# arielgabizon/barretenberg

Hardware: AMD Instinct MI355X
Metric: BN254 G1 MSM points/sec at n=2^20 (Fr NTT elems/sec in 'ntt') (higher is better)
Workload: dtype u32x9 (256-bit Montgomery, 29-bit limbs)

## Files before the change

barretenberg_amd/csrc/msm.hip:

```cpp
#include <hip/hip_runtime.h>

#include <algorithm>
#include <mutex>
#include <stdint.h>
#include <stdio.h>
#include <stdlib.h>
#include <string.h>
#include <vector>

#include "bbgpu_internal.h"
#include "g1.hpp"
#include "g1_quad.hpp"
#include "host_g1.hpp"

namespace bbgpu {

using Fr = FrP;
#define FRONT_PRIO() __builtin_amdgcn_s_setprio(2)
constexpr int TAIL_PRIO = 3;
constexpr int SCALAR_BITS = 254;
constexpr int MSM_MAX_C = 16;
constexpr int MSM_THREADS = 256;

__device__ __forceinline__ void ld8(const uint32_t* p, uint32_t (&w)[8])
{
    const uint4* q = reinterpret_cast<const uint4*>(p);
    uint4 a = q[0], b = q[1];
    w[0] = a.x; w[1] = a.y; w[2] = a.z; w[3] = a.w;
    w[4] = b.x; w[5] = b.y; w[6] = b.z; w[7] = b.w;
}
__device__ __forceinline__ void ld16(const uint32_t* p, uint32_t (&w)[16])
{
    const uint4* q = reinterpret_cast<const uint4*>(p);
#pragma unroll
    for (int i = 0; i < 4; i++) {
        uint4 a = q[i];
        w[4 * i] = a.x; w[4 * i + 1] = a.y; w[4 * i + 2] = a.z; w[4 * i + 3] = a.w;
    }
}
__device__ __forceinline__ void st32(uint32_t* p, const uint32_t (&w)[32])
{
    uint4* q = reinterpret_cast<uint4*>(p);
#pragma unroll
    for (int i = 0; i < 8; i++) q[i] = make_uint4(w[4 * i], w[4 * i + 1], w[4 * i + 2], w[4 * i + 3]);
}
__device__ __forceinline__ void ld32(const uint32_t* p, uint32_t (&w)[32])
{
    const uint4* q = reinterpret_cast<const uint4*>(p);
#pragma unroll
    for (int i = 0; i < 8; i++) {
        uint4 a = q[i];
        w[4 * i] = a.x; w[4 * i + 1] = a.y; w[4 * i + 2] = a.z; w[4 * i + 3] = a.w;
    }
}

struct WinLayout {
    uint16_t off[66];
};
static WinLayout make_layout(int c, bool balanced)
{
    WinLayout LO{};
    const int W = msm_num_windows(c);
    if (!balanced) {
        for (int w = 0; w <= W; w++) LO.off[w] = (uint16_t)(c * w);
        return LO;
    }
    const int base = SCALAR_BITS / W, rem = SCALAR_BITS - base * W;
    int bit = 0;
    for (int w = 0; w < W; w++) {
        LO.off[w] = (uint16_t)bit;
        bit += base + (w < rem ? 1 : 0);
    }
    LO.off[W] = (uint16_t)bit;
    return LO;
}
__global__ void srs_convert_kernel(const uint32_t* __restrict__ table, uint32_t* __restrict__ srs, uint32_t n, uint32_t stride_words)
{
    const uint32_t i = blockIdx.x * blockDim.x + threadIdx.x;
    if (i >= n) return;
    uint32_t w[16];
    ld16(table + (size_t)i * stride_words, w);
    AffineV<2> a;
    load_affine_m256(a, w);
    uint32_t o[16];
    store_affine_m261(o, a.x, a.y);
    uint4* q = reinterpret_cast<uint4*>(srs + (size_t)i * 16);
#pragma unroll
    for (int k = 0; k < 4; k++) q[k] = make_uint4(o[4 * k], o[4 * k + 1], o[4 * k + 2], o[4 * k + 3]);
}

// ... 71 lines not shown
    set_infinity(acc);
    for (uint32_t d = 0; d < 256; d++) {
        uint32_t o[32];
        store_xyzz(o, acc);
        st32(tab + ((size_t)w * 256 + d) * 32, o);
        Xyzz t;
        add(t, acc, base);
        acc = t;
    }
}
__device__ __forceinline__ Fe<Fq, 1, 2> fq_inverse(const Fe<Fq, 1, 2>& a)
{
    const uint64_t e[4] = { Fq::P64[0] - 2, Fq::P64[1], Fq::P64[2], Fq::P64[3] };
    return pow_u256<Fq>(a, e);
}
__global__ void srs_gen_points_kernel(const uint32_t* __restrict__ tab, Limbs9 x261, uint32_t* __restrict__ srs, uint32_t n, uint32_t first)
{
    const uint32_t i = blockIdx.x * blockDim.x + threadIdx.x;
    if (i >= n) return;
    Fe<Fr, 1, 2> s = fe_one<Fr>(), b = fe_from<Fr>(x261.d);
    for (uint32_t e = first + i; e; e >>= 1) {
        if (e & 1) s = mul(s, b);
        b = sqr(b);
    }
    uint32_t k[8];
    {
        FeT<Fr> one_raw = fe_zero<Fr>();
        one_raw.d[0] = 1;
        to_canonical(mul(s, one_raw), k);
    }
    Xyzz acc;
    set_infinity(acc);
    for (uint32_t w = 0; w < 32; w++) {
        const uint32_t d = (k[w >> 2] >> ((w & 3) * 8)) & 0xff;
        if (d) {
            uint32_t pw[32];
            ld32(tab + ((size_t)w * 256 + d) * 32, pw);
            Xyzz q;
            load_xyzz(q, pw);
            Xyzz t;
            add(t, acc, q);
            acc = t;
        }
    }
    auto inv = fq_inverse(mul(acc.zz, acc.zzz));
    auto izz = mul(inv, acc.zzz), izzz = mul(inv, acc.zz);
    uint32_t o[16];
    store_affine_m261(o, mul(acc.x, izz), mul(acc.y, izzz));
    uint4* q = reinterpret_cast<uint4*>(srs + (size_t)i * 16);
#pragma unroll
    for (int t = 0; t < 4; t++) q[t] = make_uint4(o[4 * t], o[4 * t + 1], o[4 * t + 2], o[4 * t + 3]);
}

struct ScalarSets {
    const uint32_t* p[MSM_MAX_JOBS];
};
template <class DT> struct DigitTraits { static constexpr bool wide = false; };
template <> struct DigitTraits<uint16_t> { static constexpr bool wide = true; };
template <class DT> __device__ __forceinline__ int load_digit(const DT* __restrict__ dg, const unsigned long long* __restrict__ sg, uint32_t i)
{
    if constexpr (DigitTraits<DT>::wide) {
        const int u = dg[i];
        return ((sg[i >> 6] >> (i & 63u)) & 1ull) ? -u - 1 : u;
    } else {
        return dg[i];
    }
}
template <class DT> __device__ __forceinline__ void load_digits8(const DT* __restrict__ dg, const unsigned long long* __restrict__ sg, uint32_t i8, int (&d)[8])
{
    const uint4 q = *reinterpret_cast<const uint4*>(dg + i8);
    const uint32_t w[4] = { q.x, q.y, q.z, q.w };
    if constexpr (DigitTraits<DT>::wide) {
        const uint32_t sb = reinterpret_cast<const uint8_t*>(sg)[i8 >> 3];
#pragma unroll
        for (int k = 0; k < 8; k++) {
            const int u = (int)((w[k >> 1] >> (16 * (k & 1))) & 0xffffu);
            d[k] = ((sb >> k) & 1u) ? -u - 1 : u;
        }
    } else {
#pragma unroll
        for (int k = 0; k < 8; k++) d[k] = (int)(int16_t)(w[k >> 1] >> (16 * (k & 1)));
    }
}
template <class DT> __global__ void __launch_bounds__(MSM_THREADS) msm_digits_kernel(ScalarSets sets, DT* __restrict__ digits_all, unsigned long long* __restrict__ signs_all,
                                                               uint32_t n, WinLayout LO, uint32_t num_windows, uint32_t wb, uint32_t we)
{
    FRONT_PRIO();
    const uint32_t i = blockIdx.x * blockDim.x + threadIdx.x;
    if (i >= n) return;
    const uint32_t* __restrict__ scalars = sets.p[blockIdx.y];
    DT* __restrict__ digits = digits_all + (size_t)blockIdx.y * num_windows * n;
    const uint32_t s64 = (n + 63) >> 6;
    unsigned long long* __restrict__ signs = signs_all + (size_t)blockIdx.y * num_windows * s64;
    uint32_t w[8], k[9];
    ld8(scalars + (size_t)i * 8, w);
    to_canonical(exact_limbs(mul(unpack<Fr>(w), fe_from<Fr>(Fr::M256_TO_PLAIN))), w);
#pragma unroll
    for (int j = 0; j < 8; j++) k[j] = w[j];
    k[8] = 0;
    uint32_t carry = 0;
    for (uint32_t win = 0; win < we; win++) {
        const uint32_t bit = LO.off[win], sz = LO.off[win + 1] - bit, j = bit >> 5, s = bit & 31;
        const uint32_t half = 1u << (sz - 1), mask = (1u << sz) - 1;
        uint32_t v = 0;
        if (j < 8) {
            v = k[j] >> s;
            if (s + sz > 32) v |= k[j + 1] << (32 - s);
        }
        v = (v & mask) + carry;
        carry = (win + 1 < num_windows && v >= half) ? 1u : 0u;
        const int32_t d = (int32_t)v - (int32_t)(carry << sz);
        if (win >= wb) {
            if constexpr (DigitTraits<DT>::wide) {
                const unsigned long long neg = __ballot(d < 0);
                digits[(size_t)win * n + i] = (DT)(d < 0 ? -d - 1 : d);
                if ((threadIdx.x & 63u) == 0) signs[(size_t)win * s64 + (i >> 6)] = neg;
            } else {
                digits[(size_t)win * n + i] = (DT)d;
            }
        }
    }
}

constexpr int SORT_THREADS = 1024;
constexpr uint32_t SORT_MAX_LB = 7;
constexpr uint32_t SORTB_MAX_PARTS = 8;
constexpr uint32_t SORTB_SPLIT_MIN = 1u << 16;

__device__ __forceinline__ bool wave_keys_heavy(bool valid, uint32_t key)
{
    const uint64_t vm = __ballot(valid);
    if (!vm) return false;
    const uint32_t k0 = __builtin_amdgcn_readlane(key, __ffsll((unsigned long long)vm) - 1);
    return 4 * __popcll(__ballot(valid && key == k0)) >= __popcll(vm);
}
__device__ __forceinline__ uint32_t lds_inc_dedup(uint32_t* ctr, uint32_t key, bool heavy)
{
    if (!heavy) return atomicAdd(&ctr[key], 1u);
    const uint32_t lane = __lane_id();
    uint64_t todo = __ballot(1);
    uint32_t res = 0;
    for (int it = 0; it < 4 && todo; it++) {
        const int leader = __ffsll((unsigned long long)todo) - 1;
        const uint32_t kk = __builtin_amdgcn_readlane(key, leader);
        const uint64_t m = __ballot(key == kk) & todo;
        uint32_t base = 0;
        if ((int)lane == leader) base = atomicAdd(&ctr[kk], (uint32_t)__popcll(m));
        base = __builtin_amdgcn_readlane(base, leader);
        if ((m >> lane) & 1ull) res = base + (uint32_t)__popcll(m & ((1ull << lane) - 1ull));
        todo &= ~m;
    }
    if ((todo >> lane) & 1ull) res = atomicAdd(&ctr[key], 1u);
    return res;
}

template <class DT> __global__ void __launch_bounds__(SORT_THREADS) __attribute__((amdgpu_num_vgpr(32))) sortA_hist_kernel(const DT* __restrict__ digits, const unsigned long long* __restrict__ signs, uint32_t* __restrict__ histA, uint32_t n,
                                                                uint32_t bins, uint32_t lb, uint32_t slices, uint32_t slice_len, uint32_t win0,
                                                                uint32_t wpg, uint32_t first_i0, uint32_t last_i1, uint32_t blo, uint32_t bcnt)
{
    FRONT_PRIO();
    __shared__ uint32_t lh[SORT_THREADS];
    const uint32_t s = blockIdx.x, wl = blockIdx.y;
    lh[threadIdx.x] = 0;
    __syncthreads();
    const uint32_t lo = s * slice_len, hi = min(n, lo + slice_len);
    const uint32_t s64 = (n + 63) >> 6;
    if ((n & 7u) == 0) {
        const uint32_t lo8 = lo & ~7u, bpw = lo < hi ? (((hi + 7u) & ~7u) - lo8) >> 3 : 0u;
        for (uint32_t u = threadIdx.x; u < wpg * bpw; u += SORT_THREADS) {
            const uint32_t k = u / bpw, i8 = lo8 + (u - k * bpw) * 8;
            const uint32_t klo = (k == 0) ? max(lo, first_i0) : lo, khi = (k + 1 == wpg) ? min(hi, last_i1) : hi;
            int d[8];
            load_digits8<DT>(digits + (size_t)(win0 + wl * wpg + k) * n, signs + (size_t)(win0 + wl * wpg + k) * s64, i8, d);
            const bool heavy = wave_keys_heavy(d[0] != 0, (uint32_t)((d[0] < 0 ? -d[0] : d[0]) - 1) >> lb);
#pragma unroll
            for (int j = 0; j < 8; j++)
                if (d[j] && i8 + j >= klo && i8 + j < khi) {
                    const uint32_t b = (uint32_t)((d[j] < 0 ? -d[j] : d[j]) - 1);
                    if (b - blo < bcnt) (void)lds_inc_dedup(lh, b >> lb, heavy);
                }
        }
    } else {
        for (uint32_t k = 0; k < wpg; k++) {
            const DT* dg = digits + (size_t)(win0 + wl * wpg + k) * n;
            const unsigned long long* sg = signs + (size_t)(win0 + wl * wpg + k) * s64;
            const uint32_t klo = (k == 0) ? max(lo, first_i0) : lo, khi = (k + 1 == wpg) ? min(hi, last_i1) : hi;
            for (uint32_t i = klo + threadIdx.x; i < khi; i += SORT_THREADS) {
                const int d = load_digit<DT>(dg, sg, i);
                if (d) {
                    const uint32_t b = (uint32_t)((d < 0 ? -d : d) - 1);
                    if (b - blo < bcnt) atomicAdd(&lh[b >> lb], 1u);
                }
            }
        }
    }
    __syncthreads();
    if (threadIdx.x < bins) histA[((size_t)wl * slices + s) * bins + threadIdx.x] = lh[threadIdx.x];
}

__global__ void __launch_bounds__(SORT_THREADS) sortA_colscan_kernel(uint32_t* __restrict__ histA, uint32_t* __restrict__ bintot, uint32_t bins,
                                                                   uint32_t slices)
{
    FRONT_PRIO();
    const uint32_t wl = blockIdx.y, lane = threadIdx.x & 63;
    const uint32_t bin = blockIdx.x * (SORT_THREADS / 64) + (threadIdx.x >> 6);
    if (bin >= bins) return;
    uint32_t* H = histA + (size_t)wl * slices * bins + bin;
    const uint32_t spp = (slices + 63) / 64;
    const uint32_t s0 = min(slices, lane * spp), s1 = min(slices, s0 + spp);
    uint32_t sum = 0;
    for (uint32_t s = s0; s < s1; s++) sum += H[(size_t)s * bins];
    uint32_t incl = sum;
#pragma unroll
    for (int off = 1; off < 64; off <<= 1) {
        const uint32_t v = __shfl_up(incl, off);
        if ((int)lane >= off) incl += v;
    }
    uint32_t run = incl - sum;
    for (uint32_t s = s0; s < s1; s++) {
        const uint32_t cnt = H[(size_t)s * bins];
        H[(size_t)s * bins] = run;
        run += cnt;
    }
    if (lane == 63) bintot[(size_t)wl * bins + bin] = incl;
}
__global__ void __launch_bounds__(SORT_THREADS) sortA_scan_kernel(const uint32_t* __restrict__ bintot, uint32_t* __restrict__ binstart,
                                                                uint32_t* __restrict__ totals, uint32_t bins, uint32_t* __restrict__ solo_bases,
                                                                uint32_t* __restrict__ solo_gstart_end)
{
    FRONT_PRIO();
    __shared__ uint32_t part[SORT_THREADS];
    const uint32_t wl = blockIdx.x, t = threadIdx.x;
    const uint32_t mine = t < bins ? bintot[(size_t)wl * bins + t] : 0;
    part[t] = mine;
    __syncthreads();
    for (uint32_t off = 1; off < SORT_THREADS; off <<= 1) {
        uint32_t v = t >= off ? part[t - off] : 0;
        __syncthreads();
        part[t] += v;
        __syncthreads();
    }
    if (t < bins) binstart[(size_t)wl * bins + t] = part[t] - mine;
    if (t == SORT_THREADS - 1) {
        totals[wl] = part[SORT_THREADS - 1];
        if (solo_bases) {
            solo_bases[0] = 0;
            solo_bases[1] = part[SORT_THREADS - 1];
            solo_gstart_end[0] = part[SORT_THREADS - 1];
            solo_gstart_end[1] = 0xffffffffu;
        }
    }
}
__global__ void sort_bases_kernel(const uint32_t* __restrict__ totals, uint32_t* __restrict__ bases, uint32_t* __restrict__ gstart_end, uint32_t nw)
{
    FRONT_PRIO();
    if (threadIdx.x == 0 && blockIdx.x == 0) {
        uint32_t run = 0;
        for (uint32_t w = 0; w < nw; w++) {
            bases[w] = run;
            run += totals[w];
        }
        bases[nw] = run;
        gstart_end[0] = run;
        gstart_end[1] = 0xffffffffu;
    }
}


template <class DT> __global__ void __launch_bounds__(SORT_THREADS) __attribute__((amdgpu_num_vgpr(32))) sortA_scatter_kernel(const DT* __restrict__ digits, const unsigned long long* __restrict__ signs, const uint32_t* __restrict__ cursorsA,
                                                                   const uint32_t* __restrict__ binstart, const uint32_t* __restrict__ bases,
                                                                   uint32_t* __restrict__ tmp, uint32_t n, uint32_t bins, uint32_t lb,
                                                                   uint32_t slices, uint32_t slice_len, uint32_t win0, uint32_t wpg,
                                                                   uint32_t idx_stride, uint32_t windows_per_job, uint32_t first_i0, uint32_t last_i1, uint32_t blo, uint32_t bcnt)
{
    FRONT_PRIO();
    __shared__ uint32_t lc[SORT_THREADS];
    const uint32_t s = blockIdx.x, wl = blockIdx.y;
    if (threadIdx.x < bins)
        lc[threadIdx.x] = cursorsA[((size_t)wl * slices + s) * bins + threadIdx.x] + binstart[(size_t)wl * bins + threadIdx.x] + bases[wl];
    __syncthreads();
    const uint32_t lo = s * slice_len, hi = min(n, lo + slice_len);
    const uint32_t lomask = (1u << lb) - 1;
    const uint32_t s64 = (n + 63) >> 6;
    if ((n & 7u) == 0) {
        const uint32_t lo8 = lo & ~7u, bpw = lo < hi ? (((hi + 7u) & ~7u) - lo8) >> 3 : 0u;
        for (uint32_t u = threadIdx.x; u < wpg * bpw; u += SORT_THREADS) {
            const uint32_t k = u / bpw, i8 = lo8 + (u - k * bpw) * 8;
            const uint32_t wabs = win0 + wl * wpg + k;
            const uint32_t row = (wabs % windows_per_job) * idx_stride;
            const uint32_t klo = (k == 0) ? max(lo, first_i0) : lo, khi = (k + 1 == wpg) ? min(hi, last_i1) : hi;
            int d[8];
            load_digits8<DT>(digits + (size_t)wabs * n, signs + (size_t)wabs * s64, i8, d);
#pragma unroll
            for (int j = 0; j < 8; j++) {
                if (d[j] && i8 + j >= klo && i8 + j < khi) {
                    const uint32_t b = (uint32_t)((d[j] < 0 ? -d[j] : d[j]) - 1);
                    if (b - blo < bcnt) {
                        const uint32_t pos = atomicAdd(&lc[b >> lb], 1u);
                        tmp[pos] = (row + i8 + j) | ((b & lomask) << 24) | (d[j] < 0 ? 0x80000000u : 0u);
                    }
                }
            }
        }
        return;
    }
    for (uint32_t k = 0; k < wpg; k++) {
        const uint32_t wabs = win0 + wl * wpg + k;
        const DT* dg = digits + (size_t)wabs * n;
        const unsigned long long* sg = signs + (size_t)wabs * s64;
        const uint32_t row = (wabs % windows_per_job) * idx_stride;
        const uint32_t klo = (k == 0) ? max(lo, first_i0) : lo, khi = (k + 1 == wpg) ? min(hi, last_i1) : hi;
        for (uint32_t i = klo + threadIdx.x; i < khi; i += SORT_THREADS) {
            const int d = load_digit<DT>(dg, sg, i);
            if (d) {
                const uint32_t b = (uint32_t)((d < 0 ? -d : d) - 1);
                if (b - blo < bcnt) {
                    const uint32_t pos = atomicAdd(&lc[b >> lb], 1u);
                    tmp[pos] = (row + i) | ((b & lomask) << 24) | (d < 0 ? 0x80000000u : 0u);
                }
            }
        }
    }
}

template <class DT> __global__ void __launch_bounds__(SORT_THREADS) __attribute__((amdgpu_waves_per_eu(8, 8))) sortA_scatter_staged_kernel(const DT* __restrict__ digits, const unsigned long long* __restrict__ signs, const uint32_t* __restrict__ cursorsA,
                                                                          const uint32_t* __restrict__ binstart, const uint32_t* __restrict__ bases,
                                                                          uint32_t* __restrict__ tmp, uint32_t n, uint32_t bins, uint32_t lb,
                                                                          uint32_t slices, uint32_t slice_len, uint32_t win0, uint32_t wpg,
                                                                          uint32_t idx_stride, uint32_t windows_per_job, uint32_t first_i0, uint32_t last_i1, uint32_t blo, uint32_t bcnt)
{
    FRONT_PRIO();
    constexpr uint32_t TILE = SORT_THREADS * 8;
    __shared__ uint32_t lc[SORT_THREADS];
    __shared__ uint32_t th[SORT_THREADS];
    __shared__ uint32_t dlt[SORT_THREADS];
    __shared__ uint32_t wsum[SORT_THREADS / 64 + 1];
    __shared__ uint32_t buf[TILE];
    __shared__ uint16_t bbin[TILE];
    const uint32_t s = blockIdx.x, wl = blockIdx.y, t = threadIdx.x, lane = t & 63, wave = t >> 6;
    lc[t] = t < bins ? cursorsA[((size_t)wl * slices + s) * bins + t] + binstart[(size_t)wl * bins + t] + bases[wl] : 0u;
    const uint32_t lo = s * slice_len, hi = min(n, lo + slice_len);
    const uint32_t lomask = (1u << lb) - 1;
    const uint32_t s64 = (n + 63) >> 6;
    const uint32_t lo8 = lo & ~7u, bpw = lo < hi ? (((hi + 7u) & ~7u) - lo8) >> 3 : 0u;
    const uint32_t total_u = wpg * bpw;
    for (uint32_t u0 = 0; u0 < total_u; u0 += SORT_THREADS) {
        th[t] = 0;
        __syncthreads();
        uint32_t ent[8], bn[8], rk[8];
        const uint32_t u = u0 + t;
#pragma unroll
        for (int j = 0; j < 8; j++) bn[j] = 0xffffffffu;
        if (u < total_u) {
            const uint32_t k = u / bpw, i8 = lo8 + (u - k * bpw) * 8;
            const uint32_t wabs = win0 + wl * wpg + k;
            const uint32_t row = (wabs % windows_per_job) * idx_stride;
            const uint32_t klo = (k == 0) ? max(lo, first_i0) : lo, khi = (k + 1 == wpg) ? min(hi, last_i1) : hi;
            int d[8];
            load_digits8<DT>(digits + (size_t)wabs * n, signs + (size_t)wabs * s64, i8, d);
            const bool heavy = wave_keys_heavy(d[0] != 0, (uint32_t)((d[0] < 0 ? -d[0] : d[0]) - 1) >> lb);
#pragma unroll
            for (int j = 0; j < 8; j++) {
                if (d[j] && i8 + j >= klo && i8 + j < khi) {
                    const uint32_t b = (uint32_t)((d[j] < 0 ? -d[j] : d[j]) - 1);
                    if (b - blo < bcnt) {
                        bn[j] = b >> lb;
                        ent[j] = (row + i8 + j) | ((b & lomask) << 24) | (d[j] < 0 ? 0x80000000u : 0u);
                        rk[j] = lds_inc_dedup(th, bn[j], heavy);
                    }
                }
            }
        }
        __syncthreads();
        const uint32_t c = th[t];
        uint32_t incl = c;
#pragma unroll
        for (int off = 1; off < 64; off <<= 1) {
            const uint32_t o = __shfl_up(incl, off);
            if ((int)lane >= off) incl += o;
        }
        if (lane == 63) wsum[wave] = incl;
        __syncthreads();
        uint32_t before = 0;
        for (uint32_t w = 0; w < wave; w++) before += wsum[w];
        const uint32_t excl = before + incl - c;
        th[t] = excl;
        const uint32_t g = lc[t];
        dlt[t] = g - excl;
        lc[t] = g + c;
        if (t == SORT_THREADS - 1) wsum[SORT_THREADS / 64] = excl + c;
        __syncthreads();
#pragma unroll
        for (int j = 0; j < 8; j++) {
            if (bn[j] != 0xffffffffu) {
                const uint32_t slot = th[bn[j]] + rk[j];
                buf[slot] = ent[j];
                bbin[slot] = (uint16_t)bn[j];
            }
        }
        __syncthreads();
        const uint32_t tile_n = wsum[SORT_THREADS / 64];
        for (uint32_t x = t; x < tile_n; x += SORT_THREADS) tmp[dlt[bbin[x]] + x] = buf[x];
    }
}

template <int THREADS> __global__ void __launch_bounds__(THREADS) sortB_count_kernel(const uint32_t* __restrict__ tmp, const uint32_t* __restrict__ binstart,
                                                                                       const uint32_t* __restrict__ bases, uint32_t* __restrict__ histB, uint32_t bins, uint32_t parts)
{
    FRONT_PRIO();
    constexpr int UB = 8;
    constexpr uint32_t TILE = THREADS * UB;
    __shared__ uint32_t cnt[128];
    const uint32_t bin = blockIdx.x, wl = blockIdx.y, part = blockIdx.z, t = threadIdx.x;
    const uint32_t bstart = bases[wl] + binstart[(size_t)wl * bins + bin];
    const uint32_t bend = (bin + 1 < bins) ? bases[wl] + binstart[(size_t)wl * bins + bin + 1] : bases[wl + 1];
    const uint32_t len = bend - bstart;
    if (len <= SORTB_SPLIT_MIN) return;
    const uint32_t start = bstart + (uint32_t)(((uint64_t)len * part) / parts), end = bstart + (uint32_t)(((uint64_t)len * (part + 1)) / parts);
    if (t < 128) cnt[t] = 0;
    __syncthreads();
    for (uint32_t e0 = start + t; e0 < end; e0 += TILE) {
        uint32_t v[UB];
#pragma unroll
        for (int k = 0; k < UB; k++) {
            const uint32_t e = e0 + k * THREADS;
            v[k] = e < end ? tmp[e] : 0u;
        }
        const bool heavy = wave_keys_heavy(e0 < end, (v[0] >> 24) & 0x7f);
#pragma unroll
        for (int k = 0; k < UB; k++)
            if (e0 + k * THREADS < end) (void)lds_inc_dedup(cnt, (v[k] >> 24) & 0x7f, heavy);
    }
    __syncthreads();
    if (t < 128) histB[(((size_t)wl * bins + bin) * parts + part) * 128 + t] = cnt[t];
}
template <int THREADS> __global__ void __launch_bounds__(THREADS) sortB_staged_kernel(const uint32_t* __restrict__ tmp, const uint32_t* __restrict__ binstart,
                                                                                        const uint32_t* __restrict__ bases, uint32_t* __restrict__ sorted,
                                                                                        uint32_t* __restrict__ gstart, uint32_t bins, uint32_t lb, uint32_t nb,
                                                                                        const uint32_t* __restrict__ histB, uint32_t parts_launched)
{
    FRONT_PRIO();
    constexpr int UB = 8;
    constexpr uint32_t TILE = THREADS * UB;
    __shared__ uint32_t cnt[128];
    __shared__ uint32_t cur[128];
    __shared__ uint32_t toff[128];
    __shared__ uint32_t dlt[128];
    __shared__ uint32_t bef[128];
// ... 818 lines not shown
    if (!append) {
        S.jobs = (uint32_t)jobs;
        S.n = n;
        S.pending = false;
        S.timed = false;
        S.npieces = 0;
    } else {
        S.n += n;
    }
    MsmPiece& PC = S.piece[S.npieces];
    PC = MsmPiece{};
    PC.hout_group = S.npieces ? S.piece[S.npieces - 1].hout_group + S.piece[S.npieces - 1].nw : 0u;
    if (n == 0) { PC.trivial = true; S.npieces++; S.pending = true; return BBGPU_OK; }
    if (n > ((size_t)1 << 24)) {
        set_error("MSM of %zu points: at most 2^24 points per call", n);
        return BBGPU_ERR_SIZE;
    }
    const bool hint = S.throughput;
    S.throughput = false;
    const bool table = d_tab != nullptr;
    const int c = table ? tab_c : msm_choose_c(n);
    const MsmPlan P = make_plan(n, c);
    if (wb < 0 || we > (int)P.W || wb >= we) return BBGPU_ERR_ARG;
    if (row_i1 > n) row_i1 = (uint32_t)n;
    if ((row_i0 != 0 || row_i1 != n) && (!table || jobs != 1 || row_i0 >= n || (we - wb == 1 && row_i0 >= row_i1))) return BBGPU_ERR_ARG;
    if (jobs < 1 || jobs > MSM_MAX_JOBS || (jobs > 1 && (!table || wb != 0 || we != (int)P.W))) {
        set_error("batched MSM: 1..%d jobs, window tables and the full window range required", MSM_MAX_JOBS);
        return BBGPU_ERR_ARG;
    }
    const uint32_t BH = 1u << P.hbits, BL = 1u << P.lbits;
    if (brow1 > BH) brow1 = BH;
    const bool bshare = brow0 != 0 || brow1 != BH;
    if (bshare && (!table || jobs != 1 || brow0 >= brow1 || wb != 0 || we != (int)P.W || row_i0 != 0 || row_i1 != n)) return BBGPU_ERR_ARG;
    const uint32_t blo = brow0 * BL, bcnt = (brow1 - brow0) * BL;
    const uint32_t nw1 = (uint32_t)(we - wb);
    const uint32_t nw = nw1 * (uint32_t)jobs;
    const uint32_t G = table ? (uint32_t)jobs : nw1;
    const uint32_t wpg = table ? nw1 : 1u;
    uint32_t sort_lb = P.sort_lb, sort_bins = P.sort_bins;
    if (table) {
        uint32_t want_bins = 512;
        while (sort_bins < want_bins && sort_lb > 3) { sort_lb--; sort_bins <<= 1; }
    }
    uint32_t slices = table ? std::max<uint32_t>(1, P.slices * nw1 / 2) : P.slices;
    if (table && jobs == 1) {
        const uint32_t by_cap = (uint32_t)(((uint64_t)nw * P.slices * 1024) / ((uint64_t)G * sort_bins));
        const uint32_t want = std::min<uint32_t>(std::min<uint32_t>(208, (uint32_t)(n / 2048)), by_cap);
        slices = std::max(slices, want);
    }
    const uint32_t slice_len = (uint32_t)((n + slices - 1) / slices);
    const uint32_t idx_stride = table ? (uint32_t)tab_stride : 0u;
    const uint32_t* points = table ? d_tab : d_srs;
    PC.c = P.c; PC.nw = G; PC.wb = table ? 0u : (uint32_t)wb; PC.hbits = P.hbits; PC.lbits = P.lbits;
    if (PC.hout_group + G > MSM_HOUT_GROUPS) {
        set_error("MSM in %d pieces of %u bucket sets: the result array holds %u", S.npieces + 1, G, MSM_HOUT_GROUPS);
        return BBGPU_ERR_SIZE;
    }
    int rc = ws.ensure(MsmWorkspace::bytes_needed(n, c, (int)nw, (int)G));
    if (rc) return rc;
    if (!ws.h_out) HIPCHK(hipHostMalloc((void**)&ws.h_out, (size_t)MSM_HOUT_GROUPS * 64 * 128));
    if (!S.done) HIPCHK(hipEventCreateWithFlags(&S.done, hipEventDisableTiming));

    const MsmCarve LY = carve(P, n, nw, G);
    if (LY.end > ws.cap) {
        set_error("internal: MSM workspace of %zu bytes, layout needs %zu (n=%zu c=%d nw=%u)", ws.cap, LY.end, n, c, nw);
        return BBGPU_ERR_STATE;
    }
    uint8_t* const p = ws.base;
    void* digits = (void*)(p + LY.digits);
    unsigned long long* signs = (unsigned long long*)(p + LY.signs);
    uint32_t* histA = (uint32_t*)(p + LY.histA);
    uint32_t* histB = (uint32_t*)(p + LY.histB);
    uint32_t* binstart = (uint32_t*)(p + LY.binstart);
    uint32_t* bintot = (uint32_t*)(p + LY.bintot);
    uint32_t* tmp_entries = (uint32_t*)(p + LY.tmp_entries);
    uint32_t* gstart = (uint32_t*)(p + LY.gstart);
    uint32_t* totals = (uint32_t*)(p + LY.totals);
    uint32_t* bases = totals + nw;
    uint32_t* heavy = (uint32_t*)(p + LY.heavy);
    uint32_t* sorted = (uint32_t*)(p + LY.sorted);
    uint32_t* partials = (uint32_t*)(p + LY.partials);
    uint32_t* buckets = (uint32_t*)(p + LY.buckets);
    uint32_t* scratch = (uint32_t*)(p + LY.arena);
    if ((uint64_t)G * slices * sort_bins > (uint64_t)nw * P.slices * 1024 || sort_bins > 1024 ||
        (size_t)G * ((size_t)(1u << P.hbits) + (size_t)(1u << P.lbits)) + 64 > arena_points(P, G)) {
        set_error("internal: MSM launch shape exceeds the workspace layout");
        return BBGPU_ERR_STATE;
    }

    hipEvent_t* ev = S.ev;
    const bool tm = want_timing == 1, tm_acc = want_timing != 0;
    S.timed_light = want_timing == 2;
    if (tm_acc) {
        if (!S.ev[0])
            for (int i = 0; i < 8; i++) HIPCHK(hipEventCreate(&S.ev[i]));
        if (tm) HIPCHK(hipEventRecord(ev[0], st));
        S.timed = true;
    }

    if (bshare) {
        HIPCHK(hipMemsetAsync(scratch, 0, (size_t)G * BH * 128, st));
    }
    ScalarSets sets{};
    for (int j = 0; j < jobs; j++) sets.p[j] = (const uint32_t*)d_scalars_v[j];
    const bool wide = c > 16;
    if (wide) msm_digits_kernel<uint16_t><<<dim3((P.n + MSM_THREADS - 1) / MSM_THREADS, jobs), MSM_THREADS, 0, st>>>(sets, (uint16_t*)digits, signs, P.n, make_layout(c, table), P.W, (uint32_t)wb, (uint32_t)we);
    else msm_digits_kernel<int16_t><<<dim3((P.n + MSM_THREADS - 1) / MSM_THREADS, jobs), MSM_THREADS, 0, st>>>(sets, (int16_t*)digits, signs, P.n, make_layout(c, table), P.W, (uint32_t)wb, (uint32_t)we);
    if (tm) HIPCHK(hipEventRecord(ev[1], st));
    if (wide) sortA_hist_kernel<uint16_t><<<dim3(slices, G), SORT_THREADS, 0, st>>>((const uint16_t*)digits, signs, histA, P.n, sort_bins, sort_lb, slices, slice_len, (uint32_t)wb, wpg, row_i0, row_i1, blo, bcnt);
    else sortA_hist_kernel<int16_t><<<dim3(slices, G), SORT_THREADS, 0, st>>>((const int16_t*)digits, signs, histA, P.n, sort_bins, sort_lb, slices, slice_len, (uint32_t)wb, wpg, row_i0, row_i1, blo, bcnt);
    sortA_colscan_kernel<<<dim3((sort_bins + SORT_THREADS / 64 - 1) / (SORT_THREADS / 64), G), SORT_THREADS, 0, st>>>(histA, bintot, sort_bins, slices);
    sortA_scan_kernel<<<G, SORT_THREADS, 0, st>>>(bintot, binstart, totals, sort_bins, G == 1 ? bases : nullptr, gstart + (size_t)G * P.nb);
    if (G > 1) sort_bases_kernel<<<1, 64, 0, st>>>(totals, bases, gstart + (size_t)G * P.nb, G);
    if ((P.n & 7u) == 0) {
        if (wide) sortA_scatter_staged_kernel<uint16_t><<<dim3(slices, G), SORT_THREADS, 0, st>>>((const uint16_t*)digits, signs, histA, binstart, bases, tmp_entries, P.n, sort_bins, sort_lb, slices,
                                                                                  slice_len, (uint32_t)wb, wpg, idx_stride, P.W, row_i0, row_i1, blo, bcnt);
        else sortA_scatter_staged_kernel<int16_t><<<dim3(slices, G), SORT_THREADS, 0, st>>>((const int16_t*)digits, signs, histA, binstart, bases, tmp_entries, P.n, sort_bins, sort_lb, slices,
                                                                            slice_len, (uint32_t)wb, wpg, idx_stride, P.W, row_i0, row_i1, blo, bcnt);
    } else if (wide) sortA_scatter_kernel<uint16_t><<<dim3(slices, G), SORT_THREADS, 0, st>>>((const uint16_t*)digits, signs, histA, binstart, bases, tmp_entries, P.n, sort_bins, sort_lb, slices,
                                                                   slice_len, (uint32_t)wb, wpg, idx_stride, P.W, row_i0, row_i1, blo, bcnt);
    else sortA_scatter_kernel<int16_t><<<dim3(slices, G), SORT_THREADS, 0, st>>>((const int16_t*)digits, signs, histA, binstart, bases, tmp_entries, P.n, sort_bins, sort_lb, slices,
                                                                   slice_len, (uint32_t)wb, wpg, idx_stride, P.W, row_i0, row_i1, blo, bcnt);
    if (table) {
        uint32_t parts = ((uint64_t)n * nw1 >= ((uint64_t)1 << 21) && G <= MSM_MAX_JOBS) ? SORTB_MAX_PARTS : 1u;
        if ((size_t)G * sort_bins * parts * 128 * 4 > LY.histB_bytes) parts = 1;
        if (parts > 1) sortB_count_kernel<SORT_THREADS><<<dim3(sort_bins, G, parts), SORT_THREADS, 0, st>>>(tmp_entries, binstart, bases, histB, sort_bins, parts);
        sortB_staged_kernel<SORT_THREADS><<<dim3(sort_bins, G, parts), SORT_THREADS, 0, st>>>(tmp_entries, binstart, bases, sorted, gstart, sort_bins, sort_lb, P.nb, histB, parts);
    } else sortB_staged_kernel<256><<<dim3(sort_bins, G), 256, 0, st>>>(tmp_entries, binstart, bases, sorted, gstart, sort_bins, sort_lb, P.nb, nullptr, 1u);
    if (tm_acc) HIPCHK(hipEventRecord(ev[2], st));
    const uint32_t total_buckets = G * P.nb;
    const uint64_t m_expected = bshare ? std::max<uint64_t>(1, (uint64_t)n * nw * bcnt / P.nb) : (uint64_t)n * nw;
    const uint32_t merge_buckets = bshare ? bcnt : total_buckets;
    const bool tp = hint && jobs == 1;
    constexpr uint32_t TP_MIN_CHUNK = 20;
    uint32_t ch = bshare ? chunk_len_m(m_expected) : chunk_len(n, nw);
    ch = std::max(ch, min_chunk((uint64_t)n * nw));
    if (tp && ch < TP_MIN_CHUNK)
        ch = std::max(ch, std::min<uint32_t>(TP_MIN_CHUNK, (uint32_t)(m_expected / (acc_capacity_lanes() / ACC_WG_PER_CU))));
    const uint32_t avg_partials = (uint32_t)(m_expected / ((uint64_t)merge_buckets * ch)) + 1;
    uint32_t logG = 0;
    while ((1u << logG) < avg_partials && logG < 6 && ((uint64_t)merge_buckets << (logG + 1)) <= ((uint64_t)1 << 16)) logG++;
    const uint32_t merge_light = std::max(6u, 8u << logG);
    const uint32_t max_chunks = (uint32_t)(((uint64_t)n * nw + ch - 1) / ch);
    msm_accumulate_kernel<<<(max_chunks + MSM_THREADS - 1) / MSM_THREADS, MSM_THREADS, 0, st>>>(points, sorted, gstart, partials, total_buckets, ch, 0, heavy);
    if (tm_acc) {
        HIPCHK(hipEventRecord(ev[3], st));
        if (int rc = acc_ring_record(S, st)) return rc;
    } else {
        S.acc_seq = 0;
    }
    if ((uint64_t)n * nw <= ((uint64_t)1 << 21)) {
        uint32_t logQ = 0;
        while ((2u << logQ) < avg_partials && logQ < 4 && ((uint64_t)merge_buckets << (logQ + 3)) <= ((uint64_t)1 << 17)) logQ++;
        msm_merge_quad_kernel<<<(uint32_t)((((uint64_t)merge_buckets << (logQ + 2)) + MSM_THREADS - 1) / MSM_THREADS), MSM_THREADS, 0, st>>>(gstart, partials, buckets, heavy, blo, blo + merge_buckets, ch,
                                                                                                                                  std::max(32u, 8u << logQ), logQ);
    } else msm_merge_kernel<<<(uint32_t)((((uint64_t)merge_buckets << logG) + MSM_THREADS - 1) / MSM_THREADS), MSM_THREADS, 0, st>>>(gstart, partials, buckets, heavy,
                                                                                                                     blo, blo + merge_buckets, ch, merge_light, logG);
    msm_merge_heavy_kernel<<<HEAVY_WGS, MSM_THREADS, 0, st>>>(gstart, partials, buckets, heavy, ch, heavy + (((size_t)G * P.nb + HEAVY_IDS + 63) & ~(size_t)63));
    if (tm) HIPCHK(hipEventRecord(ev[4], st));

    const uint32_t H = 1u << P.hbits, L = 1u << P.lbits;
    {
        uint32_t* Rr = scratch;
        uint32_t* Cc = scratch + (size_t)G * H * 32;
        uint32_t* const dest = (uint32_t*)ws.h_out + (size_t)PC.hout_group * 64 * 32;
        const uint32_t zero_words = G * 64 * 32;
        if (!bshare && rowcol_two_step(P) && (tp || jobs > 1)) {
            uint32_t* segs = (uint32_t*)(p + LY.segs);
            const uint32_t seg_lanes = 2 * (H * L / ROWCOL_SEG);
            msm_rowcol_seg_kernel<<<dim3((seg_lanes + MSM_THREADS - 1) / MSM_THREADS, G), MSM_THREADS, 0, st>>>(buckets, segs, H, L, dest, zero_words);
            msm_segsum_quad_kernel<<<dim3(H + L, G), 64, 0, st>>>(segs, Rr, Cc, H, L);
        } else msm_rowcol_quad_kernel<<<dim3((bshare ? brow1 - brow0 : H) + L, G), QFOLD_T, 0, st>>>(buckets, Rr, Cc, H, L, dest, zero_words, bshare ? brow0 : 0u,
                                                                                                  bshare ? brow1 - brow0 : H);
        if (tm) HIPCHK(hipEventRecord(ev[5], st));
        msm_final_quad_kernel<<<dim3(1 + P.hbits + P.lbits, G), QFOLD_T, 0, st>>>(Rr, Cc, dest, P.hbits, P.lbits);
        if (tm) HIPCHK(hipEventRecord(ev[6], st));
    }
    HIPCHK(hipEventRecord(S.done, st));
    HIPCHK(launch_check());
    S.npieces++;
    S.pending = true;
    return BBGPU_OK;
}

static host::Xyzz group_sum(const MsmSlot& S, const MsmPiece& PC, uint32_t w)
{
    auto pt = [&](uint32_t slot) {
        host::Xyzz q;
        memcpy(&q, (const uint8_t*)S.ws.h_out + ((size_t)(PC.hout_group + w) * 64 + slot) * 128, 128);
        return q;
    };
    host::Xyzz rs = host::g1_infinity();
    for (int k = (int)PC.hbits - 1; k >= 0; --k) rs = host::g1_add(host::g1_dbl(rs), pt(1 + k));
    for (uint32_t k = 0; k < PC.lbits; k++) rs = host::g1_dbl(rs);
    host::Xyzz cs = host::g1_infinity();
    for (int k = (int)PC.lbits - 1; k >= 0; --k) cs = host::g1_add(host::g1_dbl(cs), pt(32 + k));
    return host::g1_add(host::g1_add(rs, cs), pt(0));
}
static int finish_timing(MsmSlot& S, MsmTiming* timing)
{
    if (S.timed && timing) {
// ... 156 lines not shown
```

Measured before the change: 960.4 million.

## Fuse scalar digit decomposition with per-slice bucket histogram in one kernel

The digit-extraction kernel now also builds the per-slice LDS histogram of bucket bins for every window, so the separate sortA_hist pass no longer re-reads the digit and sign arrays from global memory. Blocks are reshaped to slice-by-job grids with dynamic LDS sized to rows times bins, and window offsets are broadcast via readlane. A FULL template specialisation drops bucket-range and row-bound checks when no bucket sharing or partial rows apply, also in the scatter kernel. This removes one kernel launch and a full digit read, at the cost of larger LDS per block and a new launch-shape limit on counters.

```diff
diff --git a/barretenberg_amd/csrc/msm.hip b/barretenberg_amd/csrc/msm.hip
--- a/barretenberg_amd/csrc/msm.hip
+++ b/barretenberg_amd/csrc/msm.hip
@@ -6,6 +6,7 @@
 #include <stdio.h>
 #include <stdlib.h>
 #include <string.h>
+#include <type_traits>
 #include <vector>
 
 #include "bbgpu_internal.h"
@@ -243,45 +244,6 @@
         for (int k = 0; k < 8; k++) d[k] = (int)(int16_t)(w[k >> 1] >> (16 * (k & 1)));
     }
 }
-template <class DT> __global__ void __launch_bounds__(MSM_THREADS) msm_digits_kernel(ScalarSets sets, DT* __restrict__ digits_all, unsigned long long* __restrict__ signs_all,
-                                                               uint32_t n, WinLayout LO, uint32_t num_windows, uint32_t wb, uint32_t we)
-{
-    FRONT_PRIO();
-    const uint32_t i = blockIdx.x * blockDim.x + threadIdx.x;
-    if (i >= n) return;
-    const uint32_t* __restrict__ scalars = sets.p[blockIdx.y];
-    DT* __restrict__ digits = digits_all + (size_t)blockIdx.y * num_windows * n;
-    const uint32_t s64 = (n + 63) >> 6;
-    unsigned long long* __restrict__ signs = signs_all + (size_t)blockIdx.y * num_windows * s64;
-    uint32_t w[8], k[9];
-    ld8(scalars + (size_t)i * 8, w);
-    to_canonical(exact_limbs(mul(unpack<Fr>(w), fe_from<Fr>(Fr::M256_TO_PLAIN))), w);
-#pragma unroll
-    for (int j = 0; j < 8; j++) k[j] = w[j];
-    k[8] = 0;
-    uint32_t carry = 0;
-    for (uint32_t win = 0; win < we; win++) {
-        const uint32_t bit = LO.off[win], sz = LO.off[win + 1] - bit, j = bit >> 5, s = bit & 31;
-        const uint32_t half = 1u << (sz - 1), mask = (1u << sz) - 1;
-        uint32_t v = 0;
-        if (j < 8) {
-            v = k[j] >> s;
-            if (s + sz > 32) v |= k[j + 1] << (32 - s);
-        }
-        v = (v & mask) + carry;
-        carry = (win + 1 < num_windows && v >= half) ? 1u : 0u;
-        const int32_t d = (int32_t)v - (int32_t)(carry << sz);
-        if (win >= wb) {
-            if constexpr (DigitTraits<DT>::wide) {
-                const unsigned long long neg = __ballot(d < 0);
-                digits[(size_t)win * n + i] = (DT)(d < 0 ? -d - 1 : d);
-                if ((threadIdx.x & 63u) == 0) signs[(size_t)win * s64 + (i >> 6)] = neg;
-            } else {
-                digits[(size_t)win * n + i] = (DT)d;
-            }
-        }
-    }
-}
 
 constexpr int SORT_THREADS = 1024;
 constexpr uint32_t SORT_MAX_LB = 7;
@@ -315,48 +277,80 @@
     return res;
 }
 
-template <class DT> __global__ void __launch_bounds__(SORT_THREADS) __attribute__((amdgpu_num_vgpr(32))) sortA_hist_kernel(const DT* __restrict__ digits, const unsigned long long* __restrict__ signs, uint32_t* __restrict__ histA, uint32_t n,
-                                                                uint32_t bins, uint32_t lb, uint32_t slices, uint32_t slice_len, uint32_t win0,
-                                                                uint32_t wpg, uint32_t first_i0, uint32_t last_i1, uint32_t blo, uint32_t bcnt)
+constexpr int DIGIT_THREADS = SORT_THREADS;
+constexpr uint32_t DIGIT_MAX_COUNTERS = 4096;
+template <class DT, bool FULL> __global__ void __launch_bounds__(DIGIT_THREADS) msm_digits_kernel(ScalarSets sets, DT* __restrict__ digits_all, unsigned long long* __restrict__ signs_all,
+                                                               uint32_t* __restrict__ histA, uint32_t n, WinLayout LO, uint32_t num_windows, uint32_t wb, uint32_t we,
+                                                               uint32_t bins, uint32_t lb, uint32_t slice_len, uint32_t rows,
+                                                               uint32_t first_i0, uint32_t last_i1, uint32_t blo, uint32_t bcnt)
 {
     FRONT_PRIO();
-    __shared__ uint32_t lh[SORT_THREADS];
-    const uint32_t s = blockIdx.x, wl = blockIdx.y;
-    lh[threadIdx.x] = 0;
+    extern __shared__ uint32_t lh[];
+    constexpr bool wide = DigitTraits<DT>::wide;
+    const uint32_t s = blockIdx.x, slices = gridDim.x, job = blockIdx.y;
+    for (uint32_t x = threadIdx.x; x < rows * bins; x += DIGIT_THREADS) lh[x] = 0;
     __syncthreads();
+    const uint32_t* __restrict__ scalars = sets.p[job];
+    DT* __restrict__ digits = digits_all + (size_t)job * num_windows * n;
+    const uint32_t s64 = (n + 63) >> 6;
+    unsigned long long* __restrict__ signs = signs_all + (size_t)job * num_windows * s64;
     const uint32_t lo = s * slice_len, hi = min(n, lo + slice_len);
-    const uint32_t s64 = (n + 63) >> 6;
-    if ((n & 7u) == 0) {
-        const uint32_t lo8 = lo & ~7u, bpw = lo < hi ? (((hi + 7u) & ~7u) - lo8) >> 3 : 0u;
-        for (uint32_t u = threadIdx.x; u < wpg * bpw; u += SORT_THREADS) {
-            const uint32_t k = u / bpw, i8 = lo8 + (u - k * bpw) * 8;
-            const uint32_t klo = (k == 0) ? max(lo, first_i0) : lo, khi = (k + 1 == wpg) ? min(hi, last_i1) : hi;
-            int d[8];
-            load_digits8<DT>(digits + (size_t)(win0 + wl * wpg + k) * n, signs + (size_t)(win0 + wl * wpg + k) * s64, i8, d);
-            const bool heavy = wave_keys_heavy(d[0] != 0, (uint32_t)((d[0] < 0 ? -d[0] : d[0]) - 1) >> lb);
-#pragma unroll
-            for (int j = 0; j < 8; j++)
-                if (d[j] && i8 + j >= klo && i8 + j < khi) {
-                    const uint32_t b = (uint32_t)((d[j] < 0 ? -d[j] : d[j]) - 1);
-                    if (b - blo < bcnt) (void)lds_inc_dedup(lh, b >> lb, heavy);
-                }
-        }
-    } else {
-        for (uint32_t k = 0; k < wpg; k++) {
-            const DT* dg = digits + (size_t)(win0 + wl * wpg + k) * n;
-            const unsigned long long* sg = signs + (size_t)(win0 + wl * wpg + k) * s64;
-            const uint32_t klo = (k == 0) ? max(lo, first_i0) : lo, khi = (k + 1 == wpg) ? min(hi, last_i1) : hi;
-            for (uint32_t i = klo + threadIdx.x; i < khi; i += SORT_THREADS) {
-                const int d = load_digit<DT>(dg, sg, i);
-                if (d) {
-                    const uint32_t b = (uint32_t)((d < 0 ? -d : d) - 1);
-                    if (b - blo < bcnt) atomicAdd(&lh[b >> lb], 1u);
-                }
+    const uint32_t rowstep = rows > 1 ? bins : 0u;
+    const uint32_t lane = threadIdx.x & 63u, wave0 = __builtin_amdgcn_readfirstlane(threadIdx.x & ~63u);
+    const uint32_t off_lane = LO.off[lane], off_end = __builtin_amdgcn_readfirstlane(LO.off[num_windows]);
+    for (uint32_t i0 = (wide ? lo & ~63u : lo) + wave0; i0 < hi; i0 += DIGIT_THREADS) {
+        const uint32_t i = i0 + lane;
+        const bool mine = i >= lo && i < hi;
+        const int32_t mine_mask = mine ? -1 : 0;
+        uint32_t w[8] = { 0, 0, 0, 0, 0, 0, 0, 0 }, k[9];
+        if (wide ? i < n : mine) ld8(scalars + (size_t)i * 8, w);
+        to_canonical(exact_limbs(mul(unpack<Fr>(w), fe_from<Fr>(Fr::M256_TO_PLAIN))), w);
+#pragma unroll
+        for (int j = 0; j < 8; j++) k[j] = w[j];
+        k[8] = 0;
+        uint32_t carry = 0, next = __builtin_amdgcn_readlane(off_lane, 0);
+        uint32_t* lrow = lh;
+        for (uint32_t win = 0; win < we; win++) {
+            const uint32_t bit = next;
+            next = win + 1 == num_windows ? off_end : __builtin_amdgcn_readlane(off_lane, win + 1);
+            const uint32_t sz = next - bit, j = bit >> 5, sh = bit & 31;
+            const uint32_t half = 1u << (sz - 1), mask = (1u << sz) - 1;
+            uint32_t v = 0;
+            if (j < 8) {
+                v = k[j] >> sh;
+                if (sh + sz > 32) v |= k[j + 1] << (32 - sh);
             }
+            v = (v & mask) + carry;
+            carry = (win + 1 < num_windows && v >= half) ? 1u : 0u;
+            const int32_t d = (int32_t)v - (int32_t)(carry << sz);
+            if (win < wb) continue;
+            const uint32_t mag = (uint32_t)(d < 0 ? -d - 1 : d);
+            if constexpr (wide) {
+                const unsigned long long neg = __ballot(d < 0);
+                if (mine) digits[(size_t)win * n + i] = (DT)mag;
+                if (lane == 0 && i0 >= lo) signs[(size_t)win * s64 + (i0 >> 6)] = neg;
+            } else {
+                if (mine) digits[(size_t)win * n + i] = (DT)d;
+            }
+            const uint32_t b = mag - (d > 0 ? 1u : 0u);
+            bool valid = (d & mine_mask) != 0;
+            if constexpr (!FULL) {
+                valid = valid && b - blo < bcnt;
+                if (win == wb) valid = valid && i >= first_i0;
+                if (win + 1 == we) valid = valid && i < last_i1;
+            }
+            if (valid) {
+                const uint32_t key = b >> lb;
+                (void)lds_inc_dedup(lrow, key, wave_keys_heavy(true, key));
+            }
+            lrow += rowstep;
         }
     }
     __syncthreads();
-    if (threadIdx.x < bins) histA[((size_t)wl * slices + s) * bins + threadIdx.x] = lh[threadIdx.x];
+    for (uint32_t x = threadIdx.x; x < rows * bins; x += DIGIT_THREADS) {
+        const uint32_t r = x / bins;
+        histA[((size_t)(job + r) * slices + s) * bins + (x - r * bins)] = lh[x];
+    }
 }
 
 __global__ void __launch_bounds__(SORT_THREADS) sortA_colscan_kernel(uint32_t* __restrict__ histA, uint32_t* __restrict__ bintot, uint32_t bins,
@@ -484,7 +478,7 @@
     }
 }
 
-template <class DT> __global__ void __launch_bounds__(SORT_THREADS) __attribute__((amdgpu_waves_per_eu(8, 8))) sortA_scatter_staged_kernel(const DT* __restrict__ digits, const unsigned long long* __restrict__ signs, const uint32_t* __restrict__ cursorsA,
+template <class DT, bool FULL> __global__ void __launch_bounds__(SORT_THREADS) __attribute__((amdgpu_waves_per_eu(8, 8))) sortA_scatter_staged_kernel(const DT* __restrict__ digits, const unsigned long long* __restrict__ signs, const uint32_t* __restrict__ cursorsA,
                                                                           const uint32_t* __restrict__ binstart, const uint32_t* __restrict__ bases,
                                                                           uint32_t* __restrict__ tmp, uint32_t n, uint32_t bins, uint32_t lb,
                                                                           uint32_t slices, uint32_t slice_len, uint32_t win0, uint32_t wpg,
@@ -516,7 +510,7 @@
             const uint32_t k = u / bpw, i8 = lo8 + (u - k * bpw) * 8;
             const uint32_t wabs = win0 + wl * wpg + k;
             const uint32_t row = (wabs % windows_per_job) * idx_stride;
-            const uint32_t klo = (k == 0) ? max(lo, first_i0) : lo, khi = (k + 1 == wpg) ? min(hi, last_i1) : hi;
+            const uint32_t klo = (FULL || k != 0) ? lo : max(lo, first_i0), khi = (FULL || k + 1 != wpg) ? hi : min(hi, last_i1);
             int d[8];
             load_digits8<DT>(digits + (size_t)wabs * n, signs + (size_t)wabs * s64, i8, d);
             const bool heavy = wave_keys_heavy(d[0] != 0, (uint32_t)((d[0] < 0 ? -d[0] : d[0]) - 1) >> lb);
@@ -524,7 +518,7 @@
             for (int j = 0; j < 8; j++) {
                 if (d[j] && i8 + j >= klo && i8 + j < khi) {
                     const uint32_t b = (uint32_t)((d[j] < 0 ? -d[j] : d[j]) - 1);
-                    if (b - blo < bcnt) {
+                    if (FULL || b - blo < bcnt) {
                         bn[j] = b >> lb;
                         ent[j] = (row + i8 + j) | ((b & lomask) << 24) | (d[j] < 0 ? 0x80000000u : 0u);
                         rk[j] = lds_inc_dedup(th, bn[j], heavy);
@@ -1509,7 +1503,7 @@
     uint32_t* partials = (uint32_t*)(p + LY.partials);
     uint32_t* buckets = (uint32_t*)(p + LY.buckets);
     uint32_t* scratch = (uint32_t*)(p + LY.arena);
-    if ((uint64_t)G * slices * sort_bins > (uint64_t)nw * P.slices * 1024 || sort_bins > 1024 ||
+    if ((uint64_t)G * slices * sort_bins > (uint64_t)nw * P.slices * 1024 || sort_bins > 1024 || (table ? 1u : nw1) * sort_bins > DIGIT_MAX_COUNTERS ||
         (size_t)G * ((size_t)(1u << P.hbits) + (size_t)(1u << P.lbits)) + 64 > arena_points(P, G)) {
         set_error("internal: MSM launch shape exceeds the workspace layout");
         return BBGPU_ERR_STATE;
@@ -1531,19 +1525,28 @@
     ScalarSets sets{};
     for (int j = 0; j < jobs; j++) sets.p[j] = (const uint32_t*)d_scalars_v[j];
     const bool wide = c > 16;
-    if (wide) msm_digits_kernel<uint16_t><<<dim3((P.n + MSM_THREADS - 1) / MSM_THREADS, jobs), MSM_THREADS, 0, st>>>(sets, (uint16_t*)digits, signs, P.n, make_layout(c, table), P.W, (uint32_t)wb, (uint32_t)we);
-    else msm_digits_kernel<int16_t><<<dim3((P.n + MSM_THREADS - 1) / MSM_THREADS, jobs), MSM_THREADS, 0, st>>>(sets, (int16_t*)digits, signs, P.n, make_layout(c, table), P.W, (uint32_t)wb, (uint32_t)we);
+    const uint32_t hist_rows = table ? 1u : nw1;
+    const size_t hist_lds = (size_t)hist_rows * sort_bins * 4;
+    const bool full = !bshare && row_i0 == 0 && row_i1 == n;
+    auto launch_digits = [&](auto* dg, auto is_full) {
+        using DT = std::remove_pointer_t<decltype(dg)>;
+        msm_digits_kernel<DT, decltype(is_full)::value><<<dim3(slices, jobs), DIGIT_THREADS, hist_lds, st>>>(sets, dg, signs, histA, P.n, make_layout(c, table), P.W, (uint32_t)wb, (uint32_t)we, sort_bins,
+                                                                                                      sort_lb, slice_len, hist_rows, row_i0, row_i1, blo, bcnt);
+    };
+    if (wide) full ? launch_digits((uint16_t*)digits, std::true_type{}) : launch_digits((uint16_t*)digits, std::false_type{});
+    else full ? launch_digits((int16_t*)digits, std::true_type{}) : launch_digits((int16_t*)digits, std::false_type{});
     if (tm) HIPCHK(hipEventRecord(ev[1], st));
-    if (wide) sortA_hist_kernel<uint16_t><<<dim3(slices, G), SORT_THREADS, 0, st>>>((const uint16_t*)digits, signs, histA, P.n, sort_bins, sort_lb, slices, slice_len, (uint32_t)wb, wpg, row_i0, row_i1, blo, bcnt);
-    else sortA_hist_kernel<int16_t><<<dim3(slices, G), SORT_THREADS, 0, st>>>((const int16_t*)digits, signs, histA, P.n, sort_bins, sort_lb, slices, slice_len, (uint32_t)wb, wpg, row_i0, row_i1, blo, bcnt);
     sortA_colscan_kernel<<<dim3((sort_bins + SORT_THREADS / 64 - 1) / (SORT_THREADS / 64), G), SORT_THREADS, 0, st>>>(histA, bintot, sort_bins, slices);
     sortA_scan_kernel<<<G, SORT_THREADS, 0, st>>>(bintot, binstart, totals, sort_bins, G == 1 ? bases : nullptr, gstart + (size_t)G * P.nb);
     if (G > 1) sort_bases_kernel<<<1, 64, 0, st>>>(totals, bases, gstart + (size_t)G * P.nb, G);
     if ((P.n & 7u) == 0) {
-        if (wide) sortA_scatter_staged_kernel<uint16_t><<<dim3(slices, G), SORT_THREADS, 0, st>>>((const uint16_t*)digits, signs, histA, binstart, bases, tmp_entries, P.n, sort_bins, sort_lb, slices,
-                                                                                  slice_len, (uint32_t)wb, wpg, idx_stride, P.W, row_i0, row_i1, blo, bcnt);
-        else sortA_scatter_staged_kernel<int16_t><<<dim3(slices, G), SORT_THREADS, 0, st>>>((const int16_t*)digits, signs, histA, binstart, bases, tmp_entries, P.n, sort_bins, sort_lb, slices,
-                                                                            slice_len, (uint32_t)wb, wpg, idx_stride, P.W, row_i0, row_i1, blo, bcnt);
+        auto launch_scatter = [&](auto* dg, auto is_full) {
+            using DT = std::remove_const_t<std::remove_pointer_t<decltype(dg)>>;
+            sortA_scatter_staged_kernel<DT, decltype(is_full)::value><<<dim3(slices, G), SORT_THREADS, 0, st>>>(dg, signs, histA, binstart, bases, tmp_entries, P.n, sort_bins, sort_lb, slices, slice_len,
+                                                                                                         (uint32_t)wb, wpg, idx_stride, P.W, row_i0, row_i1, blo, bcnt);
+        };
+        if (wide) full ? launch_scatter((const uint16_t*)digits, std::true_type{}) : launch_scatter((const uint16_t*)digits, std::false_type{});
+        else full ? launch_scatter((const int16_t*)digits, std::true_type{}) : launch_scatter((const int16_t*)digits, std::false_type{});
     } else if (wide) sortA_scatter_kernel<uint16_t><<<dim3(slices, G), SORT_THREADS, 0, st>>>((const uint16_t*)digits, signs, histA, binstart, bases, tmp_entries, P.n, sort_bins, sort_lb, slices,
                                                                    slice_len, (uint32_t)wb, wpg, idx_stride, P.W, row_i0, row_i1, blo, bcnt);
     else sortA_scatter_kernel<int16_t><<<dim3(slices, G), SORT_THREADS, 0, st>>>((const int16_t*)digits, signs, histA, binstart, bases, tmp_entries, P.n, sort_bins, sort_lb, slices,
```

Result: no change. 963.7 million, median of 6 (+0.3%).
